# wadewilliamsw1234/Multi-level-Indoor-SLAM

Hardware: AMD Instinct MI355X
Metric: keyframes gated/sec (VPR+kNN+LightGlue verify) (higher is better)
Workload: dtype bf16

## Files before the change

include/mlgate.h:

```cpp
#ifndef MLGATE_H
#define MLGATE_H

#include <stddef.h>
#include <stdint.h>

#ifdef __cplusplus
extern "C" {
#endif

#define MLG_OK 0
#define MLG_EINVAL (-1)
#define MLG_EHIP (-2)
#define MLG_ENOMEM (-3)

#define MLG_VIT_DEPTH 12
#define MLG_VIT_EMBED 768
#define MLG_VIT_PATCH_K 768

#define MLG_ABI_VERSION 3
#define MLG_STRUCT_INIT(T) {(uint32_t)sizeof(T), (uint32_t)MLG_ABI_VERSION}
int mlg_abi_version(void);
const char* mlg_strerror(int status);

typedef struct mlg_vit_block {
// ... 274 lines not shown
                             void* stream);
int mlg_op_mixvpr_head(const mlg_mixvpr_weights* w, const float* features, int B, float* desc, void* stream);

typedef struct mlg_sp_weights {
    uint32_t struct_size, abi_version;
    const float* conv1a_w;
    const float* conv1a_b;
    const uint16_t* w[11];
    const float* b[11];
} mlg_sp_weights;
size_t mlg_superpoint_workspace_bytes(int B, int H, int W);
int mlg_superpoint(const mlg_sp_weights* w, const uint8_t* frames, int B, int H, int W, int C, long frame_stride,
                   float detection_threshold, int max_keypoints, int nms_radius, int remove_borders, void* workspace,
                   size_t workspace_bytes, float* keypoints, float* scores, float* descriptors,
                   uint16_t* descriptors_bf16, int32_t* counts, void* stream);

typedef struct mlg_lg_block {
    const uint16_t* Wqkv; const float* bqkv;
    const uint16_t* Wout; const float* bout;
    const uint16_t* Wf1;  const float* bf1;
    const float* ln_g;    const float* ln_b;
    const uint16_t* Wf2;  const float* bf2;
} mlg_lg_block;
typedef struct mlg_lg_weights {
    uint32_t struct_size, abi_version;
    const float* Wr;
    mlg_lg_block self[9], cross[9];
    const uint16_t* Wfinal[9]; const float* bfinal[9];
    const float* wmatch[9];    const float* bmatch[9];
    const float* wconf[8];     const float* bconf[8];
// ... 131 lines not shown
```

multi-level-indoor-slam_amd/csrc/abi.cpp:

```cpp
#include <hip/hip_runtime.h>

#include <math.h>

#include <mutex>
#include <vector>

#include "../../include/mlgate.h"
#include <cstddef>

#include "common.h"
#include "kernels.h"
#include "ws_carve.h"

namespace {

constexpr int PATCH = 14;

struct VitGeom {
    int B, S, grid, P, T, Tpad, E, heads;
    explicit VitGeom(int b, int s, int e = MLG_VIT_EMBED)
        : B(b), S(s), grid(s / PATCH), P(grid * grid), T(grid * grid + 1), E(e), heads(e / 64) {
        Tpad = (T + 63) / 64 * 64;
    }
};
// ... 585 lines not shown
                                s));
    return mlg_mixvpr_head(*w, feat, B, desc, s);
}

int mlg_op_mixvpr_preprocess(const uint8_t* frames, int B, int H, int W, int C, long frame_stride, float* out,
                             void* stream) {
    return mlg_mixvpr_preprocess(frames, B, H, W, C, frame_stride, out, (hipStream_t)stream);
}

int mlg_op_mixvpr_head(const mlg_mixvpr_weights* w, const float* features, int B, float* desc, void* stream) {
    if (!mlg_head_ok(w, MLG_ABI_VERSION) || !mixvpr_head_ok(w)) return MLG_EINVAL;
    return mlg_mixvpr_head(*w, features, B, desc, (hipStream_t)stream);
}

size_t mlg_superpoint_workspace_bytes(int B, int H, int W) { return mlg_superpoint_ws_bytes(B, H, W); }

int mlg_superpoint(const mlg_sp_weights* w, const uint8_t* frames, int B, int H, int W, int C, long frame_stride,
                   float detection_threshold, int max_keypoints, int nms_radius, int remove_borders, void* workspace,
                   size_t workspace_bytes, float* keypoints, float* scores, float* descriptors,
                   uint16_t* descriptors_bf16, int32_t* counts, void* stream) {
    if (!mlg_head_ok(w, MLG_ABI_VERSION) || !frames || !workspace || !keypoints || !scores || !descriptors || !counts)
        return MLG_EINVAL;
    if (!w->conv1a_w || !w->conv1a_b) return MLG_EINVAL;
    for (int i = 0; i < 11; ++i) {
        if (!w->w[i] || !w->b[i]) return MLG_EINVAL;
        if ((reinterpret_cast<uintptr_t>(w->w[i]) & 15) || (reinterpret_cast<uintptr_t>(w->b[i]) & 15))
            return MLG_EINVAL;
    }
    if (frame_stride < (long)H * W * C) return MLG_EINVAL;
    return mlg_superpoint_run(*w, frames, B, H, W, C, frame_stride, detection_threshold, max_keypoints, nms_radius,
// ... 264 lines not shown
```

multi-level-indoor-slam_amd/csrc/kernels.h:

```cpp
#pragma once
#include <hip/hip_runtime.h>
#include <stddef.h>
#include <stdint.h>

#include <algorithm>

#include "../../include/mlgate.h"

typedef uint16_t bf16_t;

template <class T>
inline bool mlg_head_ok(const T* p, uint32_t abi_version) {
    return p && p->struct_size == (uint32_t)sizeof(T) && p->abi_version == abi_version;
}

#define MLG_PROF_SLOTS 9
struct MlgProfScope {
    int slot;
    hipStream_t s;
    double work;
    hipEvent_t a = nullptr, b = nullptr;
    MlgProfScope(int slot, hipStream_t s, double work);
    ~MlgProfScope();
};
// ... 102 lines not shown
size_t mlg_proximity_ws_bytes(int N, int nrows);
int mlg_proximity_count_run(const double* pos, const int64_t* floor, int N, int row0, int nrows, double radius,
                            int min_gap, int strict, void* ws, size_t ws_bytes, long long* totals, hipStream_t s);
int mlg_proximity_emit_run(const double* pos, const int64_t* floor, int N, int row0, int nrows, double radius,
                           int min_gap, int strict, const void* ws, size_t ws_bytes, int32_t* pairs, double* dist,
                           uint8_t* valid, hipStream_t s);

size_t mlg_ransac_ws_bytes(int P, long S_total, int H);
int mlg_ransac_run(const float* kp1, const float* kp2, const int32_t* offs, int P, long S_total, const double* K,
                   int k_stride, double thr, int H, uint64_t seed, void* ws, size_t ws_bytes, double* model_out,
                   uint8_t* mask, int32_t* inliers, double* pose, int32_t* status, hipStream_t s);
int mlg_recover_pose_run(const float* kp1, const float* kp2, const int32_t* offs, int P, const double* K,
                         int k_stride, const double* E, const uint8_t* mask, double* pose, hipStream_t s);

size_t mlg_superpoint_ws_bytes(int B, int H, int W);
int mlg_superpoint_run(const mlg_sp_weights& w, const uint8_t* frames, int B, int H, int W, int C, long frame_stride,
                       float det_thr, int max_kp, int nms_radius, int border, void* ws, size_t ws_bytes, float* kpts,
                       float* kscores, float* desc, uint16_t* desc_bf16, int32_t* count, hipStream_t s);

struct mlg_lg_conf_i {
    const int* rowseg;
    const float* wc; const float* bc;
    const float* wm; const float* bm;
    float thr, width;
    float* lz; uint8_t* flags;
};
int mlg_lg_ffn(const bf16_t* ctx, float* X, bf16_t* xcopy, int ldc, int M, const mlg_lg_block& w, hipStream_t s,
               const mlg_lg_conf_i* conf = nullptr, int relu = 0);
int mlg_lg_proj(bool self_block, const bf16_t* xcopy, int ldx, const bf16_t* W, const float* bias, const float* efac,
                const uint8_t* live, bf16_t* Q, bf16_t* K, bf16_t* Vt, int Npad, hipStream_t s);
// ... 42 lines not shown
```

multi-level-indoor-slam_amd/csrc/superpoint.hip:

```cpp
#include "common.h"
#include "kernels.h"
#include "model_shapes.h"
#include "ws_carve.h"

namespace {

constexpr int TS = 16;
constexpr int HALO = TS + 2;
constexpr int KC = 64;

__global__ __launch_bounds__(256) void k_sp_conv1a(const uint8_t* __restrict__ frames, long frame_stride, int H, int W,
                                                   int C, const float* __restrict__ w, const float* __restrict__ b,
                                                   bf16_t* __restrict__ out) {
    __shared__ float g[HALO][HALO];
    __shared__ float sw[64 * 9 + 64];
    const int bz = blockIdx.z;
    const int y0 = blockIdx.y * TS, x0 = blockIdx.x * TS;
    const uint8_t* img = frames + (size_t)bz * frame_stride;
    for (int i = threadIdx.x; i < 64 * 9; i += 256) sw[i] = w[i];
    if (threadIdx.x < 64) sw[576 + threadIdx.x] = b[threadIdx.x];
    for (int i = threadIdx.x; i < HALO * HALO; i += 256) {
        const int yy = y0 - 1 + i / HALO, xx = x0 - 1 + i % HALO;
        float v = 0.f;
        if (yy >= 0 && yy < H && xx >= 0 && xx < W) {
// ... 243 lines not shown
    const long i = (long)blockIdx.x * blockDim.x + threadIdx.x;
    if (i < n) mask[i] = mask[i] | ((ss[i] == mp[i]) & !supp[i]);
}
__global__ void k_nms_final(float* __restrict__ s, const uint8_t* __restrict__ mask, int B, int H, int W,
                            int border) {
    const long i = (long)blockIdx.x * blockDim.x + threadIdx.x;
    if (i >= (long)B * H * W) return;
    const int x = (int)(i % W), y = (int)((i / W) % H);
    float v = mask[i] ? s[i] : 0.f;
    if (y < border || x < border || y >= H - border || x >= W - border) v = -1.f;
    s[i] = v;
}

constexpr int NMS_TH = 32, NMS_TW = 64, NMS_HALO = 20;
constexpr int NMS_LH = NMS_TH + 2 * NMS_HALO, NMS_LW = NMS_TW + 2 * NMS_HALO, NMS_N = NMS_LH * NMS_LW;

template <typename T> struct Vec4;
template <> struct Vec4<float> { typedef float4 type; };
template <> struct Vec4<uint8_t> { typedef uchar4 type; };

template <typename T>
__device__ __forceinline__ T vmax_(T a, T b) { return a > b ? a : b; }
template <>
__device__ __forceinline__ float vmax_(float a, float b) { return fmaxf(a, b); }

template <int M, typename T>
__device__ __forceinline__ void nms_pool4(const T* in, T* tmp, T* out, T lo) {
    typedef typename Vec4<T>::type V;
    constexpr int GX = NMS_LW / 4, GY = NMS_LH / 4;
    constexpr int XR0 = M > 4 ? M - 4 : 0, XR1 = M > 4 ? NMS_LH - M + 4 : NMS_LH;
    constexpr int XG0 = M / 4, XGN = GX - 2 * (M / 4);
    for (int i = threadIdx.x; i < (XR1 - XR0) * XGN; i += blockDim.x) {
        const int y = XR0 + i / XGN, g = XG0 + i % XGN;
        const V* row = reinterpret_cast<const V*>(in + y * NMS_LW);
        const V c = row[g];
        const V l = g > 0 ? row[g - 1] : V{lo, lo, lo, lo};
        const V r = g + 1 < GX ? row[g + 1] : V{lo, lo, lo, lo};
        const T v[12] = {l.x, l.y, l.z, l.w, c.x, c.y, c.z, c.w, r.x, r.y, r.z, r.w};
        T o[4];
#pragma unroll
        for (int k = 0; k < 4; ++k) {
            T m = v[k];
#pragma unroll
            for (int d = 1; d <= 8; ++d) m = vmax_(m, v[k + d]);
            o[k] = m;
        }
        reinterpret_cast<V*>(tmp + y * NMS_LW)[g] = V{o[0], o[1], o[2], o[3]};
    }
    __syncthreads();
    constexpr int YG0 = M / 4, YGN = GY - 2 * (M / 4), YC0 = M, YCN = NMS_LW - 2 * M;
    for (int i = threadIdx.x; i < YGN * YCN; i += blockDim.x) {
        const int g = YG0 + i / YCN, x = YC0 + i % YCN, y0 = 4 * g;
        T v[12];
#pragma unroll
        for (int k = 0; k < 12; ++k) {
            const int y = y0 - 4 + k;
            v[k] = (y >= 0 && y < NMS_LH) ? tmp[y * NMS_LW + x] : lo;
        }
#pragma unroll
        for (int k = 0; k < 4; ++k) {
            T m = v[k];
#pragma unroll
            for (int d = 1; d <= 8; ++d) m = vmax_(m, v[k + d]);
            out[(y0 + k) * NMS_LW + x] = m;
        }
    }
    __syncthreads();
}

__global__ __launch_bounds__(512) void k_sp_nms(const float* __restrict__ sc, float* __restrict__ out, int B, int H,
                                                int W, int border) {
    __shared__ __attribute__((aligned(16))) char nms_smem[(size_t)NMS_N * (4 * 4 + 3)];
    float* S = reinterpret_cast<float*>(nms_smem);
    float* A = S + NMS_N;
    float* Tm = A + NMS_N;
    float* P = Tm + NMS_N;
    uint8_t* MK = reinterpret_cast<uint8_t*>(P + NMS_N);
    uint8_t* SP = MK + NMS_N;
    uint8_t* TU = SP + NMS_N;
    const int tx = blockIdx.x, ty = blockIdx.y, b = blockIdx.z;
    const int ox = tx * NMS_TW - NMS_HALO, oy = ty * NMS_TH - NMS_HALO;
    const float* img = sc + (size_t)b * H * W;
    auto inside = [&](int i) {
        const int y = i / NMS_LW + oy, x = i % NMS_LW + ox;
        return y >= 0 && y < H && x >= 0 && x < W;
    };
    for (int i = threadIdx.x; i < NMS_N; i += blockDim.x) {
        const int y = i / NMS_LW + oy, x = i % NMS_LW + ox;
        S[i] = (y >= 0 && y < H && x >= 0 && x < W) ? img[(size_t)y * W + x] : -INFINITY;
    }
    __syncthreads();
    nms_pool4<4>(S, Tm, P, -INFINITY);
    for (int i = threadIdx.x; i < NMS_N; i += blockDim.x) MK[i] = inside(i) && S[i] == P[i];
    __syncthreads();
    auto iteration = [&](auto m) {
        constexpr int MS = decltype(m)::value;
        nms_pool4<MS + 4>(MK, TU, SP, (uint8_t)0);
        for (int i = threadIdx.x; i < NMS_N; i += blockDim.x) A[i] = inside(i) ? (SP[i] ? 0.f : S[i]) : -INFINITY;
        __syncthreads();
        nms_pool4<MS + 8>(A, Tm, P, -INFINITY);
        for (int i = threadIdx.x; i < NMS_N; i += blockDim.x)
            MK[i] = MK[i] | (inside(i) && A[i] == P[i] && !SP[i]);
        __syncthreads();
    };
    iteration(std::integral_constant<int, 4>{});
    iteration(std::integral_constant<int, 12>{});
    for (int i = threadIdx.x; i < NMS_TH * NMS_TW; i += blockDim.x) {
        const int ly = i / NMS_TW + NMS_HALO, lx = i % NMS_TW + NMS_HALO;
        const int y = ly + oy, x = lx + ox;
        if (y >= H || x >= W) continue;
        const int l = ly * NMS_LW + lx;
        float v = MK[l] ? S[l] : 0.f;
        if (y < border || x < border || y >= H - border || x >= W - border) v = -1.f;
        out[(size_t)b * H * W + (size_t)y * W + x] = v;
    }
}

constexpr int SEL_T = 1024;
constexpr int SEL_KMAX = 4096;

__global__ __launch_bounds__(SEL_T) void k_sp_select(const float* __restrict__ scores, int H, int W, float thr, int k,
                                                     uint32_t* __restrict__ cand_key, int32_t* __restrict__ cand_idx,
                                                     float* __restrict__ kpts, float* __restrict__ kscore,
                                                     int32_t* __restrict__ count) {
    const int b = blockIdx.x, tid = threadIdx.x;
    const long HW = (long)H * W;
    const float* s = scores + b * HW;
    uint32_t* ck = cand_key + b * HW;
    int32_t* ci = cand_idx + b * HW;
    __shared__ int scan[SEL_T];
    __shared__ uint32_t hist[256];
    __shared__ unsigned long long keys[SEL_KMAX];
    __shared__ int sh_n, sh_gt;
    __shared__ uint32_t sh_prefix;

    __shared__ int wsum[2][SEL_T / 64];
    const int lane = tid & 63, wave = tid >> 6;
    constexpr int PER = 16, CH = SEL_T * PER;
    const bool vec = (HW & 3) == 0;
    int base = 0;
    for (long c0 = 0, it = 0; c0 < HW; c0 += CH, ++it) {
        const long p0 = c0 + (long)tid * PER;
        float v[PER];
#pragma unroll
        for (int q = 0; q < PER / 4; ++q) {
            const long i = p0 + 4 * q;
            if (vec && i + 3 < HW) {
                const float4 f = *reinterpret_cast<const float4*>(s + i);
                v[4 * q] = f.x; v[4 * q + 1] = f.y; v[4 * q + 2] = f.z; v[4 * q + 3] = f.w;
            } else {
#pragma unroll
                for (int j = 0; j < 4; ++j) v[4 * q + j] = i + j < HW ? s[i + j] : -INFINITY;
            }
        }
        int cnt = 0;
#pragma unroll
        for (int j = 0; j < PER; ++j) cnt += v[j] > thr;
        int x = cnt;
#pragma unroll
        for (int o = 1; o < 64; o <<= 1) {
            const int y = __shfl_up(x, o, 64);
            if (lane >= o) x += y;
        }
        if (lane == 63) wsum[it & 1][wave] = x;
        __syncthreads();
        int wbase = 0, tot = 0;
#pragma unroll
        for (int w = 0; w < SEL_T / 64; ++w) {
            const int t = wsum[it & 1][w];
            wbase += w < wave ? t : 0;
            tot += t;
        }
        int off = base + wbase + x - cnt;
#pragma unroll
        for (int j = 0; j < PER; ++j)
            if (v[j] > thr) {
                ck[off] = __float_as_uint(v[j]);
                ci[off] = (int32_t)(p0 + j);
                ++off;
            }
        base += tot;
    }
    if (tid == 0) sh_n = base;
    __syncthreads();
    const int n = sh_n;
    float* kp = kpts + (size_t)b * k * 2;
    float* ks = kscore + (size_t)b * k;
    if (n <= k) {
        for (int i = tid; i < n; i += SEL_T) {
            const int idx = ci[i];
            kp[2 * i] = (float)(idx % W);
            kp[2 * i + 1] = (float)(idx / W);
            ks[i] = __uint_as_float(ck[i]);
        }
        if (tid == 0) count[b] = n;
        return;
    }
    uint32_t prefix = 0, pmask = 0;
    int want = k;
    for (int pass = 0; pass < 4; ++pass) {
        const int shift = 24 - 8 * pass;
        if (tid < 256) hist[tid] = 0;
        __syncthreads();
        for (int i = tid; i < n; i += SEL_T) {
            const uint32_t key = ck[i];
            if ((key & pmask) == prefix) atomicAdd(&hist[(key >> shift) & 255], 1u);
        }
        __syncthreads();
        if (tid == 0) {
            int acc = 0, d = 255;
            for (; d > 0; --d) {
                if (acc + (int)hist[d] >= want) break;
                acc += hist[d];
            }
            sh_prefix = prefix | ((uint32_t)d << shift);
            sh_gt = acc;
        }
        __syncthreads();
        want -= sh_gt;
        prefix = sh_prefix;
        pmask |= 255u << shift;
        __syncthreads();
    }
    const uint32_t T = prefix;
    if (tid == 0) sh_gt = 0;
    __syncthreads();
    int gt = 0;
    for (int i = tid; i < n; i += SEL_T) gt += ck[i] > T;
    atomicAdd(&sh_gt, gt);
    __syncthreads();
    const int need_eq = k - sh_gt;
    const int seg2 = (n + SEL_T - 1) / SEL_T;
    const int b0 = tid * seg2, b1 = min(n, b0 + seg2);
    int e = 0;
    for (int i = b0; i < b1; ++i) e += ck[i] == T;
    scan[tid] = e;
    __syncthreads();
    for (int o = 1; o < SEL_T; o <<= 1) {
        const int v = tid >= o ? scan[tid - o] : 0;
        __syncthreads();
        scan[tid] += v;
        __syncthreads();
    }
    if (tid == 0) sh_n = 0;
    __syncthreads();
    int erank = scan[tid] - e;
    for (int i = b0; i < b1; ++i) {
        const uint32_t key = ck[i];
        bool take = key > T;
        if (key == T) {
            take = erank < need_eq;
            ++erank;
        }
        if (take) {
            const int slot = atomicAdd(&sh_n, 1);
            keys[slot] = ((unsigned long long)key << 32) | (uint32_t)(~(uint32_t)ci[i]);
        }
    }
    __syncthreads();
    int np2 = 1;
    while (np2 < k) np2 <<= 1;
    for (int i = k + tid; i < np2; i += SEL_T) keys[i] = 0ull;
    __syncthreads();
    for (int size = 2; size <= np2; size <<= 1)
        for (int stride = size >> 1; stride > 0; stride >>= 1) {
            for (int i = tid; i < np2; i += SEL_T) {
                const int j = i ^ stride;
                if (j > i) {
                    const bool desc = (i & size) == 0;
                    const unsigned long long a = keys[i], bq = keys[j];
                    if ((a < bq) == desc) { keys[i] = bq; keys[j] = a; }
                }
            }
            __syncthreads();
        }
    for (int i = tid; i < k; i += SEL_T) {
        const unsigned long long v = keys[i];
        const int idx = (int)(~(uint32_t)(v & 0xffffffffu));
        kp[2 * i] = (float)(idx % W);
        kp[2 * i + 1] = (float)(idx / W);
        ks[i] = __uint_as_float((uint32_t)(v >> 32));
    }
    if (tid == 0) count[b] = k;
}

__device__ __forceinline__ float4 cell_normed(const float* __restrict__ d, const float* __restrict__ bias, int lane,
                                              bool valid) {
    if (!valid) return make_float4(0.f, 0.f, 0.f, 0.f);
    float4 v = *reinterpret_cast<const float4*>(d + lane * 4);
    const float4 bb = *reinterpret_cast<const float4*>(bias + lane * 4);
// ... 79 lines not shown
template <int L>
int gemm_layer(const mlg_sp_weights& w, const bf16_t* in, float* out, int M, hipStream_t s) {
    constexpr SpLayer l = SP_LAYERS[L];
    static_assert(l.k == 1, "gemm_layer is the 1 x 1 kernel");
    return mlg_gemm_f32out(in, w.w[L], out, M, l.cout, l.cin, s);
}

struct SpBufs {
    bf16_t *A, *Bf;
    float *logits, *dmap, *sc;
    float *t0, *t1;
    uint8_t* mask;
    uint8_t *u0, *u1;
    uint32_t* ckey;
    int32_t* cidx;
};

size_t sp_carve(int B, int H, int W, void* base, SpBufs* out) {
    WsCarver c(base);
    SpBufs b;
    const size_t n = (size_t)B * H * W, cells = (size_t)H * W / 64;
    b.A = c.take<bf16_t>(n * 64);
    b.Bf = c.take<bf16_t>(n * 64);
    b.logits = c.take<float>(B * cells * 128);
    b.dmap = c.take<float>(B * cells * 256);
    b.sc = c.take<float>(n);
    b.t0 = c.take<float>(2 * n);
    b.t1 = b.t0 ? b.t0 + n : nullptr;
    b.mask = c.take<uint8_t>(n);
    b.u0 = c.take<uint8_t>(2 * n);
    b.u1 = b.u0 ? b.u0 + n : nullptr;
    b.ckey = c.take<uint32_t>(n);
    b.cidx = c.take<int32_t>(n);
    if (out) *out = b;
    return c.total();
}

}

size_t mlg_superpoint_ws_bytes(int B, int H, int W) {
    if (B <= 0 || H < 16 || W < 16) return 0;
    return sp_carve(B, H, W, nullptr, nullptr);
}

int mlg_superpoint_run(const mlg_sp_weights& w, const uint8_t* frames, int B, int H, int W, int C, long frame_stride,
                       float det_thr, int max_kp, int nms_radius, int border, void* ws, size_t ws_bytes, float* kpts,
                       float* kscores, float* desc, uint16_t* desc_bf16, int32_t* count, hipStream_t s) {
    if (B <= 0 || H < 16 || W < 16 || (C != 1 && C != 3 && C != 4) || max_kp <= 0 ||
        max_kp > SEL_KMAX || nms_radius < 0 || border < 0)
        return MLG_EINVAL;
    SpBufs b;
    if (sp_carve(B, H, W, ws, &b) > ws_bytes) return MLG_EINVAL;
// ... 7 lines not shown
    MLG_TRY((conv_layer<1, false>(w, b.Bf, b.A, B, h, wd, s)));
    MLG_TRY((conv_layer<2, true>(w, b.A, b.Bf, B, h, wd, s)));
    h /= 2; wd /= 2;
    MLG_TRY((conv_layer<3, false>(w, b.Bf, b.A, B, h, wd, s)));
    MLG_TRY((conv_layer<4, true>(w, b.A, b.Bf, B, h, wd, s)));
    h /= 2; wd /= 2;
    MLG_TRY((conv_layer<5, false>(w, b.Bf, b.A, B, h, wd, s)));
    MLG_TRY((conv_layer<6, false>(w, b.A, b.Bf, B, h, wd, s)));
    const int M = B * h * wd;
    bf16_t* cPa = b.A;
    bf16_t* cDa = b.A + (size_t)M * SP_LAYERS[7].cout;
    MLG_TRY((conv_layer<7, false>(w, b.Bf, cPa, B, h, wd, s)));
    MLG_TRY((conv_layer<9, false>(w, b.Bf, cDa, B, h, wd, s)));
    MLG_TRY((gemm_layer<8>(w, cPa, b.logits, M, s)));
    MLG_TRY((gemm_layer<10>(w, cDa, b.dmap, M, s)));
    hipLaunchKernelGGL(k_sp_scores, dim3((M + 255) / 256), dim3(256), 0, s, b.logits, 128, w.b[8], B, h, wd, b.sc);
    MLG_LAUNCH_CHECK();
    H = 8 * h;
    W = 8 * wd;
    const float* nms_out = b.sc;
    if (nms_radius == 4) {
        hipLaunchKernelGGL(k_sp_nms, dim3((unsigned)((W + NMS_TW - 1) / NMS_TW), (unsigned)((H + NMS_TH - 1) / NMS_TH),
                                          (unsigned)B),
                           dim3(512), 0, s, b.sc, b.t0, B, H, W, border);
        MLG_LAUNCH_CHECK();
        nms_out = b.t0;
    } else {
        const long n = (long)B * H * W;
        const dim3 g((unsigned)((n + 255) / 256)), t(256);
        auto maxpool_f = [&](const float* in, float* out) {
            hipLaunchKernelGGL(k_maxfilt<float>, g, t, 0, s, in, b.t1, B, H, W, nms_radius, 0);
            hipLaunchKernelGGL(k_maxfilt<float>, g, t, 0, s, (const float*)b.t1, out, B, H, W, nms_radius, 1);
        };
        maxpool_f(b.sc, b.t0);
        hipLaunchKernelGGL(k_nms_init, g, t, 0, s, b.sc, b.t0, b.mask, n);
        for (int it = 0; it < 2; ++it) {
            hipLaunchKernelGGL(k_maxfilt<uint8_t>, g, t, 0, s, b.mask, b.u1, B, H, W, nms_radius, 0);
            hipLaunchKernelGGL(k_maxfilt<uint8_t>, g, t, 0, s, (const uint8_t*)b.u1, b.u0, B, H, W, nms_radius, 1);
            hipLaunchKernelGGL(k_nms_supp, g, t, 0, s, b.sc, b.u0, b.t0, n);
            hipLaunchKernelGGL(k_maxfilt<float>, g, t, 0, s, (const float*)b.t0, b.t1, B, H, W, nms_radius, 0);
            float* mp = (float*)b.ckey;
            hipLaunchKernelGGL(k_maxfilt<float>, g, t, 0, s, (const float*)b.t1, mp, B, H, W, nms_radius, 1);
            hipLaunchKernelGGL(k_nms_update, g, t, 0, s, b.t0, mp, b.u0, b.mask, n);
        }
        hipLaunchKernelGGL(k_nms_final, g, t, 0, s, b.sc, b.mask, B, H, W, border);
        MLG_LAUNCH_CHECK();
    }
    hipLaunchKernelGGL(k_sp_select, dim3(B), dim3(SEL_T), 0, s, nms_out, H, W, det_thr, max_kp, b.ckey, b.cidx, kpts,
                       kscores, count);
    MLG_LAUNCH_CHECK();
    hipLaunchKernelGGL(k_sp_desc, dim3((unsigned)(((long)B * max_kp + 3) / 4)), dim3(256), 0, s, b.dmap, w.b[10], B, h,
                       wd, kpts, count, max_kp, desc, desc_bf16);
    MLG_LAUNCH_CHECK();
    return MLG_OK;
}
```

multi-level-indoor-slam_amd/mlgate/_native.py:

```python
import ctypes
import os

_HERE = os.path.dirname(os.path.abspath(__file__))
LIB_PATH = os.path.join(_HERE, "libmlgate.so")
TORCH_LIB_PATH = os.path.join(_HERE, "libmlgate_torch.so")
OPS = ("vit_forward_into", "dino_forward_into", "dino_weights_check", "salad_forward", "knn_gate", "knn_query", "row_normalize", "similarity", "xcorr_score", "xcorr_batch", "rerank_gate", "seq_gate",
       "knn_append", "superpoint",
       "lightglue", "ransac_epipolar", "recover_pose", "resnet50", "loftr_features", "loftr_pack_tails", "loftr_coarse_layer", "loftr_match", "superglue", "pillow_resize_224", "plane_ransac", "proximity",
       "jpeg_pixels", "mixvpr_forward", "mixvpr_head", "mixvpr_preprocess", "vlad", "anyloc_forward", "kmeans_step",
       "crica_forward", "vit_trunk", "crica_pool", "crica_encoder",
       "weights_check", "prof_enable", "prof_reset", "prof_read")


c_int, c_long, c_size_t, c_float, c_double, c_void_p = (
    ctypes.c_int, ctypes.c_long, ctypes.c_size_t, ctypes.c_float, ctypes.c_double, ctypes.c_void_p)

EXPORTS = {
    "mlg_abi_version": (c_int, []),
    "mlg_strerror": (ctypes.c_char_p, [c_int]),
    "mlg_vit_workspace_bytes": (c_size_t, [c_int, c_int]),
    "mlg_vit_forward": (c_int, [c_void_p, c_void_p, c_int, c_int, c_int, c_int, c_long, c_int, c_int, c_void_p,
                                c_size_t, c_void_p, c_void_p, c_void_p]),
    "mlg_dino_workspace_bytes": (c_size_t, [c_int, c_int, c_int]),
    "mlg_dino_forward": (c_int, [c_void_p, c_void_p, c_int, c_int, c_int, c_int, c_long, c_int, c_int, c_void_p,
# ... 42 lines not shown
    "mlg_anyloc_workspace_bytes": (c_size_t, [c_int, c_int, c_int]),
    "mlg_anyloc_forward": (c_int, [c_void_p, c_void_p, c_void_p, c_int, c_int, c_int, c_int, c_long, c_int, c_int,
                                   c_void_p, c_size_t, c_void_p, c_void_p]),
    "mlg_kmeans_workspace_bytes": (c_size_t, [c_long, c_int]),
    "mlg_kmeans_step": (c_int, [c_void_p, c_long, c_void_p, c_int, c_void_p, c_void_p, c_void_p, c_void_p, c_size_t,
                                c_void_p]),
    "mlg_crica_forward": (c_int, [c_void_p, c_void_p, c_void_p, c_int, c_int, c_int, c_int, c_long, c_int, c_int,
                                  c_int, c_void_p, c_size_t, c_void_p, c_void_p, c_void_p]),
    "mlg_op_vit_trunk": (c_int, [c_void_p, c_void_p, c_int, c_int, c_int, c_int, c_long, c_int, c_int, c_void_p,
                                 c_size_t, c_void_p, c_void_p]),
    "mlg_op_crica_pool": (c_int, [c_void_p, c_void_p, c_void_p, c_int, c_int, c_float, c_void_p, c_void_p]),
    "mlg_op_crica_encoder": (c_int, [c_void_p, c_void_p, c_int, c_int, c_void_p, c_size_t, c_void_p, c_void_p]),
    "mlg_superpoint_workspace_bytes": (c_size_t, [c_int, c_int, c_int]),
    "mlg_superpoint": (c_int, [c_void_p, c_void_p, c_int, c_int, c_int, c_int, c_long, c_float, c_int, c_int, c_int,
                               c_void_p, c_size_t, c_void_p, c_void_p, c_void_p, c_void_p, c_void_p, c_void_p]),
    "mlg_lightglue_workspace_bytes": (c_size_t, [c_int, c_int]),
    "mlg_lightglue": (c_int, [c_void_p, c_void_p, c_void_p, c_void_p, c_int, c_int, c_void_p, c_void_p, c_int,
                              c_float, c_float, c_float, c_int, c_void_p, c_size_t, c_void_p, c_void_p, c_void_p,
                              c_void_p, c_void_p]),
    "mlg_op_gemm_f32out": (c_int, [c_void_p, c_void_p, c_void_p, c_int, c_int, c_int, c_void_p]),
    "mlg_op_gemm_f32out_variant": (c_int, [c_int, c_void_p, c_void_p, c_void_p, c_int, c_int, c_int, c_void_p]),
    "mlg_set_gemm_variant": (c_int, [c_int]),
    "mlg_set_loftr_similarity": (c_int, [c_int]),
    "mlg_op_gemm_bias_gelu": (c_int, [c_void_p, c_void_p, c_void_p, c_void_p, c_int, c_int, c_int, c_void_p]),
    "mlg_op_gemm_residual": (c_int, [c_void_p, c_void_p, c_void_p, c_void_p, c_void_p, c_int, c_int, c_int,
                                     c_void_p]),
    "mlg_op_gemm_residual_split": (c_int, [c_void_p, c_void_p, c_void_p, c_void_p, c_void_p, c_int, c_int, c_int,
                                           c_void_p]),
    "mlg_op_gemm_bias_gelu_split": (c_int, [c_void_p, c_void_p, c_void_p, c_void_p, c_int, c_int, c_int, c_void_p]),
    "mlg_op_layernorm_bf16": (c_int, [c_void_p, c_void_p, c_void_p, c_void_p, c_int, c_void_p]),
# ... 144 lines not shown
```

Measured before the change: 551.7.

## Fuse SuperPoint softmax, NMS and candidate emission into one tiled kernel

```diff
diff --git a/include/mlgate.h b/include/mlgate.h
--- a/include/mlgate.h
+++ b/include/mlgate.h
@@ -312,6 +312,7 @@
                    float detection_threshold, int max_keypoints, int nms_radius, int remove_borders, void* workspace,
                    size_t workspace_bytes, float* keypoints, float* scores, float* descriptors,
                    uint16_t* descriptors_bf16, int32_t* counts, void* stream);
+int mlg_set_superpoint_tail(int tail);
 
 typedef struct mlg_lg_block {
     const uint16_t* Wqkv; const float* bqkv;
diff --git a/multi-level-indoor-slam_amd/csrc/abi.cpp b/multi-level-indoor-slam_amd/csrc/abi.cpp
--- a/multi-level-indoor-slam_amd/csrc/abi.cpp
+++ b/multi-level-indoor-slam_amd/csrc/abi.cpp
@@ -623,6 +623,7 @@
 }
 
 size_t mlg_superpoint_workspace_bytes(int B, int H, int W) { return mlg_superpoint_ws_bytes(B, H, W); }
+int mlg_set_superpoint_tail(int tail) { return mlg_superpoint_set_tail(tail); }
 
 int mlg_superpoint(const mlg_sp_weights* w, const uint8_t* frames, int B, int H, int W, int C, long frame_stride,
                    float detection_threshold, int max_keypoints, int nms_radius, int remove_borders, void* workspace,
diff --git a/multi-level-indoor-slam_amd/csrc/kernels.h b/multi-level-indoor-slam_amd/csrc/kernels.h
--- a/multi-level-indoor-slam_amd/csrc/kernels.h
+++ b/multi-level-indoor-slam_amd/csrc/kernels.h
@@ -140,6 +140,7 @@
                          int k_stride, const double* E, const uint8_t* mask, double* pose, hipStream_t s);
 
 size_t mlg_superpoint_ws_bytes(int B, int H, int W);
+int mlg_superpoint_set_tail(int tail);
 int mlg_superpoint_run(const mlg_sp_weights& w, const uint8_t* frames, int B, int H, int W, int C, long frame_stride,
                        float det_thr, int max_kp, int nms_radius, int border, void* ws, size_t ws_bytes, float* kpts,
                        float* kscores, float* desc, uint16_t* desc_bf16, int32_t* count, hipStream_t s);
diff --git a/multi-level-indoor-slam_amd/csrc/superpoint.hip b/multi-level-indoor-slam_amd/csrc/superpoint.hip
--- a/multi-level-indoor-slam_amd/csrc/superpoint.hip
+++ b/multi-level-indoor-slam_amd/csrc/superpoint.hip
@@ -281,6 +281,11 @@
 
 constexpr int NMS_TH = 32, NMS_TW = 64, NMS_HALO = 20;
 constexpr int NMS_LH = NMS_TH + 2 * NMS_HALO, NMS_LW = NMS_TW + 2 * NMS_HALO, NMS_N = NMS_LH * NMS_LW;
+static_assert(NMS_HALO % 8 == 4 && NMS_TH % 8 == 0 && NMS_TW % 8 == 0, "cells of a tile");
+constexpr int NMS_CH = NMS_LH / 8 + 1, NMS_CW = NMS_LW / 8 + 1, NMS_CELLS = NMS_CH * NMS_CW;
+constexpr size_t NMS_LDS_BYTES = (size_t)NMS_N * (4 + 4 + 1 + 1);
+static_assert(NMS_LDS_BYTES + 2 * NMS_CELLS * 4 + 64 <= 80 * 1024, "two workgroups per CU");
+static_assert((size_t)NMS_TH * NMS_TW * 8 <= (size_t)NMS_N * 4, "candidate staging fits the scratch plane");
 
 template <typename T> struct Vec4;
 template <> struct Vec4<float> { typedef float4 type; };
@@ -291,18 +296,17 @@
 template <>
 __device__ __forceinline__ float vmax_(float a, float b) { return fmaxf(a, b); }
 
-template <int M, typename T>
-__device__ __forceinline__ void nms_pool4(const T* in, T* tmp, T* out, T lo) {
+template <int M, typename T, typename Load, typename Emit>
+__device__ __forceinline__ void nms_pool4(Load load, T* tmp, T lo, Emit emit) {
     typedef typename Vec4<T>::type V;
     constexpr int GX = NMS_LW / 4, GY = NMS_LH / 4;
     constexpr int XR0 = M > 4 ? M - 4 : 0, XR1 = M > 4 ? NMS_LH - M + 4 : NMS_LH;
     constexpr int XG0 = M / 4, XGN = GX - 2 * (M / 4);
     for (int i = threadIdx.x; i < (XR1 - XR0) * XGN; i += blockDim.x) {
         const int y = XR0 + i / XGN, g = XG0 + i % XGN;
-        const V* row = reinterpret_cast<const V*>(in + y * NMS_LW);
-        const V c = row[g];
-        const V l = g > 0 ? row[g - 1] : V{lo, lo, lo, lo};
-        const V r = g + 1 < GX ? row[g + 1] : V{lo, lo, lo, lo};
+        const V c = load(y, g);
+        const V l = g > 0 ? load(y, g - 1) : V{lo, lo, lo, lo};
+        const V r = g + 1 < GX ? load(y, g + 1) : V{lo, lo, lo, lo};
         const T v[12] = {l.x, l.y, l.z, l.w, c.x, c.y, c.z, c.w, r.x, r.y, r.z, r.w};
         T o[4];
 #pragma unroll
@@ -329,49 +333,106 @@
             T m = v[k];
 #pragma unroll
             for (int d = 1; d <= 8; ++d) m = vmax_(m, v[k + d]);
-            out[(y0 + k) * NMS_LW + x] = m;
+            emit(y0 + k, x, m);
         }
     }
     __syncthreads();
 }
 
-__global__ __launch_bounds__(512) void k_sp_nms(const float* __restrict__ sc, float* __restrict__ out, int B, int H,
-                                                int W, int border) {
-    __shared__ __attribute__((aligned(16))) char nms_smem[(size_t)NMS_N * (4 * 4 + 3)];
+template <bool LOGITS, bool EMIT>
+__global__ __launch_bounds__(512, 2) void k_sp_nms(const float* __restrict__ src, int ld,
+                                                   const float* __restrict__ bias, float* __restrict__ out, int B,
+                                                   int H, int W, int border, float thr,
+                                                   uint32_t* __restrict__ cand_key, int32_t* __restrict__ cand_idx,
+                                                   int32_t* __restrict__ cand_n) {
+    __shared__ __attribute__((aligned(16))) char nms_smem[NMS_LDS_BYTES];
+    __shared__ float cmx[NMS_CELLS], csum[NMS_CELLS];
+    __shared__ int sh_cand, sh_base;
     float* S = reinterpret_cast<float*>(nms_smem);
-    float* A = S + NMS_N;
-    float* Tm = A + NMS_N;
-    float* P = Tm + NMS_N;
-    uint8_t* MK = reinterpret_cast<uint8_t*>(P + NMS_N);
+    float* T = S + NMS_N;
+    uint8_t* TU = reinterpret_cast<uint8_t*>(T);
+    uint8_t* MK = reinterpret_cast<uint8_t*>(T + NMS_N);
     uint8_t* SP = MK + NMS_N;
-    uint8_t* TU = SP + NMS_N;
     const int tx = blockIdx.x, ty = blockIdx.y, b = blockIdx.z;
     const int ox = tx * NMS_TW - NMS_HALO, oy = ty * NMS_TH - NMS_HALO;
-    const float* img = sc + (size_t)b * H * W;
-    auto inside = [&](int i) {
-        const int y = i / NMS_LW + oy, x = i % NMS_LW + ox;
+    if (threadIdx.x == 0) sh_cand = 0;
+    if (LOGITS) {
+        const int Hc = H / 8, Wc = W / 8, cy0 = oy >> 3, cx0 = ox >> 3;
+        const float* lg = src + (size_t)b * Hc * Wc * ld;
+        if (threadIdx.x < NMS_CELLS) {
+            const int cy = cy0 + threadIdx.x / NMS_CW, cx = cx0 + threadIdx.x % NMS_CW;
+            if (cy >= 0 && cy < Hc && cx >= 0 && cx < Wc) {
+                const float* l = lg + ((size_t)cy * Wc + cx) * ld;
+                float v[65];
+                float mx = -INFINITY;
+#pragma unroll
+                for (int c = 0; c < 65; ++c) {
+                    v[c] = l[c] + bias[c];
+                    mx = fmaxf(mx, v[c]);
+                }
+                float s = 0.f;
+#pragma unroll
+                for (int c = 0; c < 65; ++c) {
+                    v[c] = expf(v[c] - mx);
+                    s += v[c];
+                }
+                cmx[threadIdx.x] = mx;
+                csum[threadIdx.x] = s;
+            }
+        }
+        __syncthreads();
+        for (int i = threadIdx.x; i < NMS_CELLS * 64; i += blockDim.x) {
+            const int cell = i >> 6, c = i & 63;
+            const int cy = cy0 + cell / NMS_CW, cx = cx0 + cell % NMS_CW;
+            const int ly = cy * 8 + (c >> 3) - oy, lx = cx * 8 + (c & 7) - ox;
+            if (ly < 0 || ly >= NMS_LH || lx < 0 || lx >= NMS_LW) continue;
+            float sc = -INFINITY;
+            if (cy >= 0 && cy < Hc && cx >= 0 && cx < Wc) {
+                const float v = lg[((size_t)cy * Wc + cx) * ld + c] + bias[c];
+                sc = expf(v - cmx[cell]) / csum[cell];
+            }
+            S[ly * NMS_LW + lx] = sc;
+        }
+    } else {
+        const float* img = src + (size_t)b * H * W;
+        for (int i = threadIdx.x; i < NMS_N; i += blockDim.x) {
+            const int y = i / NMS_LW + oy, x = i % NMS_LW + ox;
+            S[i] = (y >= 0 && y < H && x >= 0 && x < W) ? img[(size_t)y * W + x] : -INFINITY;
+        }
+    }
+    __syncthreads();
+    auto inside = [&](int ly, int lx) {
+        const int y = ly + oy, x = lx + ox;
         return y >= 0 && y < H && x >= 0 && x < W;
     };
-    for (int i = threadIdx.x; i < NMS_N; i += blockDim.x) {
-        const int y = i / NMS_LW + oy, x = i % NMS_LW + ox;
-        S[i] = (y >= 0 && y < H && x >= 0 && x < W) ? img[(size_t)y * W + x] : -INFINITY;
-    }
-    __syncthreads();
-    nms_pool4<4>(S, Tm, P, -INFINITY);
-    for (int i = threadIdx.x; i < NMS_N; i += blockDim.x) MK[i] = inside(i) && S[i] == P[i];
-    __syncthreads();
+    auto load_s = [&](int y, int g) { return reinterpret_cast<const float4*>(S + y * NMS_LW)[g]; };
+    auto load_mk = [&](int y, int g) { return reinterpret_cast<const uchar4*>(MK + y * NMS_LW)[g]; };
+    auto load_a = [&](int y, int g) {
+        float4 s = load_s(y, g);
+        const uchar4 p = reinterpret_cast<const uchar4*>(SP + y * NMS_LW)[g];
+        const int lx = 4 * g;
+        if (p.x && inside(y, lx)) s.x = 0.f;
+        if (p.y && inside(y, lx + 1)) s.y = 0.f;
+        if (p.z && inside(y, lx + 2)) s.z = 0.f;
+        if (p.w && inside(y, lx + 3)) s.w = 0.f;
+        return s;
+    };
+    nms_pool4<4, float>(load_s, T, -INFINITY, [&](int y, int x, float m) {
+        const int l = y * NMS_LW + x;
+        MK[l] = inside(y, x) && S[l] == m;
+    });
     auto iteration = [&](auto m) {
         constexpr int MS = decltype(m)::value;
-        nms_pool4<MS + 4>(MK, TU, SP, (uint8_t)0);
-        for (int i = threadIdx.x; i < NMS_N; i += blockDim.x) A[i] = inside(i) ? (SP[i] ? 0.f : S[i]) : -INFINITY;
-        __syncthreads();
-        nms_pool4<MS + 8>(A, Tm, P, -INFINITY);
-        for (int i = threadIdx.x; i < NMS_N; i += blockDim.x)
-            MK[i] = MK[i] | (inside(i) && A[i] == P[i] && !SP[i]);
-        __syncthreads();
+        nms_pool4<MS + 4, uint8_t>(load_mk, TU, (uint8_t)0,
+                                   [&](int y, int x, uint8_t mm) { SP[y * NMS_LW + x] = mm; });
+        nms_pool4<MS + 8, float>(load_a, T, -INFINITY, [&](int y, int x, float mm) {
+            const int l = y * NMS_LW + x;
+            MK[l] = MK[l] | (inside(y, x) && !SP[l] && S[l] == mm);
+        });
     };
     iteration(std::integral_constant<int, 4>{});
     iteration(std::integral_constant<int, 12>{});
+    uint2* stage = reinterpret_cast<uint2*>(T);
     for (int i = threadIdx.x; i < NMS_TH * NMS_TW; i += blockDim.x) {
         const int ly = i / NMS_TW + NMS_HALO, lx = i % NMS_TW + NMS_HALO;
         const int y = ly + oy, x = lx + ox;
@@ -379,155 +440,35 @@
         const int l = ly * NMS_LW + lx;
         float v = MK[l] ? S[l] : 0.f;
         if (y < border || x < border || y >= H - border || x >= W - border) v = -1.f;
-        out[(size_t)b * H * W + (size_t)y * W + x] = v;
+        if (EMIT) {
+            if (v > thr) stage[atomicAdd(&sh_cand, 1)] = make_uint2(__float_as_uint(v), (uint32_t)(y * W + x));
+        } else {
+            out[(size_t)b * H * W + (size_t)y * W + x] = v;
+        }
+    }
+    if (EMIT) {
+        __syncthreads();
+        const int n = sh_cand;
+        if (threadIdx.x == 0 && n > 0) sh_base = atomicAdd(&cand_n[b], n);
+        __syncthreads();
+        if (n > 0) {
+            const size_t base = (size_t)b * H * W + sh_base;
+            for (int i = threadIdx.x; i < n; i += blockDim.x) {
+                cand_key[base + i] = stage[i].x;
+                cand_idx[base + i] = (int32_t)stage[i].y;
+            }
+        }
     }
 }
 
 constexpr int SEL_T = 1024;
 constexpr int SEL_KMAX = 4096;
 
-__global__ __launch_bounds__(SEL_T) void k_sp_select(const float* __restrict__ scores, int H, int W, float thr, int k,
-                                                     uint32_t* __restrict__ cand_key, int32_t* __restrict__ cand_idx,
-                                                     float* __restrict__ kpts, float* __restrict__ kscore,
-                                                     int32_t* __restrict__ count) {
-    const int b = blockIdx.x, tid = threadIdx.x;
-    const long HW = (long)H * W;
-    const float* s = scores + b * HW;
-    uint32_t* ck = cand_key + b * HW;
-    int32_t* ci = cand_idx + b * HW;
-    __shared__ int scan[SEL_T];
-    __shared__ uint32_t hist[256];
-    __shared__ unsigned long long keys[SEL_KMAX];
-    __shared__ int sh_n, sh_gt;
-    __shared__ uint32_t sh_prefix;
-
-    __shared__ int wsum[2][SEL_T / 64];
-    const int lane = tid & 63, wave = tid >> 6;
-    constexpr int PER = 16, CH = SEL_T * PER;
-    const bool vec = (HW & 3) == 0;
-    int base = 0;
-    for (long c0 = 0, it = 0; c0 < HW; c0 += CH, ++it) {
-        const long p0 = c0 + (long)tid * PER;
-        float v[PER];
-#pragma unroll
-        for (int q = 0; q < PER / 4; ++q) {
-            const long i = p0 + 4 * q;
-            if (vec && i + 3 < HW) {
-                const float4 f = *reinterpret_cast<const float4*>(s + i);
-                v[4 * q] = f.x; v[4 * q + 1] = f.y; v[4 * q + 2] = f.z; v[4 * q + 3] = f.w;
-            } else {
-#pragma unroll
-                for (int j = 0; j < 4; ++j) v[4 * q + j] = i + j < HW ? s[i + j] : -INFINITY;
-            }
-        }
-        int cnt = 0;
-#pragma unroll
-        for (int j = 0; j < PER; ++j) cnt += v[j] > thr;
-        int x = cnt;
-#pragma unroll
-        for (int o = 1; o < 64; o <<= 1) {
-            const int y = __shfl_up(x, o, 64);
-            if (lane >= o) x += y;
-        }
-        if (lane == 63) wsum[it & 1][wave] = x;
-        __syncthreads();
-        int wbase = 0, tot = 0;
-#pragma unroll
-        for (int w = 0; w < SEL_T / 64; ++w) {
-            const int t = wsum[it & 1][w];
-            wbase += w < wave ? t : 0;
-            tot += t;
-        }
-        int off = base + wbase + x - cnt;
-#pragma unroll
-        for (int j = 0; j < PER; ++j)
-            if (v[j] > thr) {
-                ck[off] = __float_as_uint(v[j]);
-                ci[off] = (int32_t)(p0 + j);
-                ++off;
-            }
-        base += tot;
-    }
-    if (tid == 0) sh_n = base;
-    __syncthreads();
-    const int n = sh_n;
-    float* kp = kpts + (size_t)b * k * 2;
-    float* ks = kscore + (size_t)b * k;
-    if (n <= k) {
-        for (int i = tid; i < n; i += SEL_T) {
-            const int idx = ci[i];
-            kp[2 * i] = (float)(idx % W);
-            kp[2 * i + 1] = (float)(idx / W);
-            ks[i] = __uint_as_float(ck[i]);
-        }
-        if (tid == 0) count[b] = n;
-        return;
-    }
-    uint32_t prefix = 0, pmask = 0;
-    int want = k;
-    for (int pass = 0; pass < 4; ++pass) {
-        const int shift = 24 - 8 * pass;
-        if (tid < 256) hist[tid] = 0;
-        __syncthreads();
-        for (int i = tid; i < n; i += SEL_T) {
-            const uint32_t key = ck[i];
-            if ((key & pmask) == prefix) atomicAdd(&hist[(key >> shift) & 255], 1u);
-        }
-        __syncthreads();
-        if (tid == 0) {
-            int acc = 0, d = 255;
-            for (; d > 0; --d) {
-                if (acc + (int)hist[d] >= want) break;
-                acc += hist[d];
-            }
-            sh_prefix = prefix | ((uint32_t)d << shift);
-            sh_gt = acc;
-        }
-        __syncthreads();
-        want -= sh_gt;
-        prefix = sh_prefix;
-        pmask |= 255u << shift;
-        __syncthreads();
-    }
-    const uint32_t T = prefix;
-    if (tid == 0) sh_gt = 0;
-    __syncthreads();
-    int gt = 0;
-    for (int i = tid; i < n; i += SEL_T) gt += ck[i] > T;
-    atomicAdd(&sh_gt, gt);
-    __syncthreads();
-    const int need_eq = k - sh_gt;
-    const int seg2 = (n + SEL_T - 1) / SEL_T;
-    const int b0 = tid * seg2, b1 = min(n, b0 + seg2);
-    int e = 0;
-    for (int i = b0; i < b1; ++i) e += ck[i] == T;
-    scan[tid] = e;
-    __syncthreads();
-    for (int o = 1; o < SEL_T; o <<= 1) {
-        const int v = tid >= o ? scan[tid - o] : 0;
-        __syncthreads();
-        scan[tid] += v;
-        __syncthreads();
-    }
-    if (tid == 0) sh_n = 0;
-    __syncthreads();
-    int erank = scan[tid] - e;
-    for (int i = b0; i < b1; ++i) {
-        const uint32_t key = ck[i];
-        bool take = key > T;
-        if (key == T) {
-            take = erank < need_eq;
-            ++erank;
-        }
-        if (take) {
-            const int slot = atomicAdd(&sh_n, 1);
-            keys[slot] = ((unsigned long long)key << 32) | (uint32_t)(~(uint32_t)ci[i]);
-        }
-    }
-    __syncthreads();
+__device__ __forceinline__ void sel_sort_desc(unsigned long long* keys, int n) {
+    const int tid = threadIdx.x;
     int np2 = 1;
-    while (np2 < k) np2 <<= 1;
-    for (int i = k + tid; i < np2; i += SEL_T) keys[i] = 0ull;
+    while (np2 < n) np2 <<= 1;
+    for (int i = n + tid; i < np2; i += SEL_T) keys[i] = 0ull;
     __syncthreads();
     for (int size = 2; size <= np2; size <<= 1)
         for (int stride = size >> 1; stride > 0; stride >>= 1) {
@@ -541,6 +482,140 @@
             }
             __syncthreads();
         }
+}
+
+template <bool LIST>
+__global__ __launch_bounds__(SEL_T) void k_sp_select(const float* __restrict__ scores,
+                                                     const int32_t* __restrict__ cand_n, int H, int W, float thr,
+                                                     int k, uint32_t* __restrict__ cand_key,
+                                                     int32_t* __restrict__ cand_idx, float* __restrict__ kpts,
+                                                     float* __restrict__ kscore, int32_t* __restrict__ count) {
+    const int b = blockIdx.x, tid = threadIdx.x;
+    const long HW = (long)H * W;
+    uint32_t* ck = cand_key + b * HW;
+    int32_t* ci = cand_idx + b * HW;
+    __shared__ uint32_t hist[256];
+    __shared__ unsigned long long keys[SEL_KMAX];
+    __shared__ int sh_n, sh_gt;
+    __shared__ unsigned long long sh_prefix;
+    int n;
+    if (LIST) {
+        n = cand_n[b];
+    } else {
+        const float* s = scores + b * HW;
+        __shared__ int wsum[2][SEL_T / 64];
+        const int lane = tid & 63, wave = tid >> 6;
+        constexpr int PER = 16, CH = SEL_T * PER;
+        const bool vec = (HW & 3) == 0;
+        int base = 0;
+        for (long c0 = 0, it = 0; c0 < HW; c0 += CH, ++it) {
+            const long p0 = c0 + (long)tid * PER;
+            float v[PER];
+#pragma unroll
+            for (int q = 0; q < PER / 4; ++q) {
+                const long i = p0 + 4 * q;
+                if (vec && i + 3 < HW) {
+                    const float4 f = *reinterpret_cast<const float4*>(s + i);
+                    v[4 * q] = f.x; v[4 * q + 1] = f.y; v[4 * q + 2] = f.z; v[4 * q + 3] = f.w;
+                } else {
+#pragma unroll
+                    for (int j = 0; j < 4; ++j) v[4 * q + j] = i + j < HW ? s[i + j] : -INFINITY;
+                }
+            }
+            int cnt = 0;
+#pragma unroll
+            for (int j = 0; j < PER; ++j) cnt += v[j] > thr;
+            int x = cnt;
+#pragma unroll
+            for (int o = 1; o < 64; o <<= 1) {
+                const int y = __shfl_up(x, o, 64);
+                if (lane >= o) x += y;
+            }
+            if (lane == 63) wsum[it & 1][wave] = x;
+            __syncthreads();
+            int wbase = 0, tot = 0;
+#pragma unroll
+            for (int w = 0; w < SEL_T / 64; ++w) {
+                const int t = wsum[it & 1][w];
+                wbase += w < wave ? t : 0;
+                tot += t;
+            }
+            int off = base + wbase + x - cnt;
+#pragma unroll
+            for (int j = 0; j < PER; ++j)
+                if (v[j] > thr) {
+                    ck[off] = __float_as_uint(v[j]);
+                    ci[off] = (int32_t)(p0 + j);
+                    ++off;
+                }
+            base += tot;
+        }
+        if (tid == 0) sh_n = base;
+        __syncthreads();
+        n = sh_n;
+    }
+    float* kp = kpts + (size_t)b * k * 2;
+    float* ks = kscore + (size_t)b * k;
+    auto sort_key = [&](int i) { return ((unsigned long long)ck[i] << 32) | (uint32_t)(~(uint32_t)ci[i]); };
+    if (n <= k) {
+        if (LIST) {
+            for (int i = tid; i < n; i += SEL_T)
+                keys[i] = ((unsigned long long)(~(uint32_t)ci[i]) << 32) | ck[i];
+            __syncthreads();
+            sel_sort_desc(keys, n);
+            for (int i = tid; i < n; i += SEL_T) {
+                const unsigned long long v = keys[i];
+                const int idx = (int)(~(uint32_t)(v >> 32));
+                kp[2 * i] = (float)(idx % W);
+                kp[2 * i + 1] = (float)(idx / W);
+                ks[i] = __uint_as_float((uint32_t)(v & 0xffffffffu));
+            }
+        } else {
+            for (int i = tid; i < n; i += SEL_T) {
+                const int idx = ci[i];
+                kp[2 * i] = (float)(idx % W);
+                kp[2 * i + 1] = (float)(idx / W);
+                ks[i] = __uint_as_float(ck[i]);
+            }
+        }
+        if (tid == 0) count[b] = n;
+        return;
+    }
+    unsigned long long prefix = 0, pmask = 0;
+    int want = k;
+    for (int pass = 0; pass < 8; ++pass) {
+        const int shift = 56 - 8 * pass;
+        if (tid < 256) hist[tid] = 0;
+        __syncthreads();
+        for (int i = tid; i < n; i += SEL_T) {
+            const unsigned long long key = sort_key(i);
+            if ((key & pmask) == prefix) atomicAdd(&hist[(uint32_t)(key >> shift) & 255], 1u);
+        }
+        __syncthreads();
+        if (tid == 0) {
+            int acc = 0, d = 255;
+            for (; d > 0; --d) {
+                if (acc + (int)hist[d] >= want) break;
+                acc += hist[d];
+            }
+            sh_prefix = prefix | ((unsigned long long)d << shift);
+            sh_gt = acc;
+        }
+        __syncthreads();
+        want -= sh_gt;
+        prefix = sh_prefix;
+        pmask |= 255ull << shift;
+        __syncthreads();
+    }
+    const unsigned long long T = prefix;
+    if (tid == 0) sh_n = 0;
+    __syncthreads();
+    for (int i = tid; i < n; i += SEL_T) {
+        const unsigned long long key = sort_key(i);
+        if (key >= T) keys[atomicAdd(&sh_n, 1)] = key;
+    }
+    __syncthreads();
+    sel_sort_desc(keys, k);
     for (int i = tid; i < k; i += SEL_T) {
         const unsigned long long v = keys[i];
         const int idx = (int)(~(uint32_t)(v & 0xffffffffu));
@@ -650,6 +725,7 @@
     uint8_t *u0, *u1;
     uint32_t* ckey;
     int32_t* cidx;
+    int32_t* ccnt;
 };
 
 size_t sp_carve(int B, int H, int W, void* base, SpBufs* out) {
@@ -668,10 +744,19 @@
     b.u1 = b.u0 ? b.u0 + n : nullptr;
     b.ckey = c.take<uint32_t>(n);
     b.cidx = c.take<int32_t>(n);
+    b.ccnt = reinterpret_cast<int32_t*>(b.sc);
     if (out) *out = b;
     return c.total();
 }
 
+int g_tail = 0;
+
+}
+
+int mlg_superpoint_set_tail(int tail) {
+    if (tail != 0 && tail != 1) return MLG_EINVAL;
+    g_tail = tail;
+    return MLG_OK;
 }
 
 size_t mlg_superpoint_ws_bytes(int B, int H, int W) {
@@ -709,41 +794,51 @@
     MLG_TRY((conv_layer<9, false>(w, b.Bf, cDa, B, h, wd, s)));
     MLG_TRY((gemm_layer<8>(w, cPa, b.logits, M, s)));
     MLG_TRY((gemm_layer<10>(w, cDa, b.dmap, M, s)));
-    hipLaunchKernelGGL(k_sp_scores, dim3((M + 255) / 256), dim3(256), 0, s, b.logits, 128, w.b[8], B, h, wd, b.sc);
-    MLG_LAUNCH_CHECK();
     H = 8 * h;
     W = 8 * wd;
-    const float* nms_out = b.sc;
-    if (nms_radius == 4) {
-        hipLaunchKernelGGL(k_sp_nms, dim3((unsigned)((W + NMS_TW - 1) / NMS_TW), (unsigned)((H + NMS_TH - 1) / NMS_TH),
-                                          (unsigned)B),
-                           dim3(512), 0, s, b.sc, b.t0, B, H, W, border);
+    const dim3 nms_grid((unsigned)((W + NMS_TW - 1) / NMS_TW), (unsigned)((H + NMS_TH - 1) / NMS_TH), (unsigned)B);
+    if (nms_radius == 4 && g_tail == 0) {
+        if (hipMemsetAsync(b.ccnt, 0, sizeof(int32_t) * B, s) != hipSuccess) return MLG_EHIP;
+        hipLaunchKernelGGL((k_sp_nms<true, true>), nms_grid, dim3(512), 0, s, b.logits, 128, w.b[8], nullptr, B, H, W,
+                           border, det_thr, b.ckey, b.cidx, b.ccnt);
         MLG_LAUNCH_CHECK();
-        nms_out = b.t0;
+        hipLaunchKernelGGL(k_sp_select<true>, dim3(B), dim3(SEL_T), 0, s, nullptr, b.ccnt, H, W, det_thr, max_kp,
+                           b.ckey, b.cidx, kpts, kscores, count);
+        MLG_LAUNCH_CHECK();
     } else {
-        const long n = (long)B * H * W;
-        const dim3 g((unsigned)((n + 255) / 256)), t(256);
-        auto maxpool_f = [&](const float* in, float* out) {
-            hipLaunchKernelGGL(k_maxfilt<float>, g, t, 0, s, in, b.t1, B, H, W, nms_radius, 0);
-            hipLaunchKernelGGL(k_maxfilt<float>, g, t, 0, s, (const float*)b.t1, out, B, H, W, nms_radius, 1);
-        };
-        maxpool_f(b.sc, b.t0);
-        hipLaunchKernelGGL(k_nms_init, g, t, 0, s, b.sc, b.t0, b.mask, n);
-        for (int it = 0; it < 2; ++it) {
-            hipLaunchKernelGGL(k_maxfilt<uint8_t>, g, t, 0, s, b.mask, b.u1, B, H, W, nms_radius, 0);
-            hipLaunchKernelGGL(k_maxfilt<uint8_t>, g, t, 0, s, (const uint8_t*)b.u1, b.u0, B, H, W, nms_radius, 1);
-            hipLaunchKernelGGL(k_nms_supp, g, t, 0, s, b.sc, b.u0, b.t0, n);
-            hipLaunchKernelGGL(k_maxfilt<float>, g, t, 0, s, (const float*)b.t0, b.t1, B, H, W, nms_radius, 0);
-            float* mp = (float*)b.ckey;
-            hipLaunchKernelGGL(k_maxfilt<float>, g, t, 0, s, (const float*)b.t1, mp, B, H, W, nms_radius, 1);
-            hipLaunchKernelGGL(k_nms_update, g, t, 0, s, b.t0, mp, b.u0, b.mask, n);
-        }
-        hipLaunchKernelGGL(k_nms_final, g, t, 0, s, b.sc, b.mask, B, H, W, border);
+        hipLaunchKernelGGL(k_sp_scores, dim3((M + 255) / 256), dim3(256), 0, s, b.logits, 128, w.b[8], B, h, wd, b.sc);
         MLG_LAUNCH_CHECK();
-    }
-    hipLaunchKernelGGL(k_sp_select, dim3(B), dim3(SEL_T), 0, s, nms_out, H, W, det_thr, max_kp, b.ckey, b.cidx, kpts,
-                       kscores, count);
-    MLG_LAUNCH_CHECK();
+        const float* nms_out = b.sc;
+        if (nms_radius == 4) {
+            hipLaunchKernelGGL((k_sp_nms<false, false>), nms_grid, dim3(512), 0, s, b.sc, 0, nullptr, b.t0, B, H, W,
+                               border, det_thr, nullptr, nullptr, nullptr);
+            MLG_LAUNCH_CHECK();
+            nms_out = b.t0;
+        } else {
+            const long n = (long)B * H * W;
+            const dim3 g((unsigned)((n + 255) / 256)), t(256);
+            auto maxpool_f = [&](const float* in, float* out) {
+                hipLaunchKernelGGL(k_maxfilt<float>, g, t, 0, s, in, b.t1, B, H, W, nms_radius, 0);
+                hipLaunchKernelGGL(k_maxfilt<float>, g, t, 0, s, (const float*)b.t1, out, B, H, W, nms_radius, 1);
+            };
+            maxpool_f(b.sc, b.t0);
+            hipLaunchKernelGGL(k_nms_init, g, t, 0, s, b.sc, b.t0, b.mask, n);
+            for (int it = 0; it < 2; ++it) {
+                hipLaunchKernelGGL(k_maxfilt<uint8_t>, g, t, 0, s, b.mask, b.u1, B, H, W, nms_radius, 0);
+                hipLaunchKernelGGL(k_maxfilt<uint8_t>, g, t, 0, s, (const uint8_t*)b.u1, b.u0, B, H, W, nms_radius, 1);
+                hipLaunchKernelGGL(k_nms_supp, g, t, 0, s, b.sc, b.u0, b.t0, n);
+                hipLaunchKernelGGL(k_maxfilt<float>, g, t, 0, s, (const float*)b.t0, b.t1, B, H, W, nms_radius, 0);
+                float* mp = (float*)b.ckey;
+                hipLaunchKernelGGL(k_maxfilt<float>, g, t, 0, s, (const float*)b.t1, mp, B, H, W, nms_radius, 1);
+                hipLaunchKernelGGL(k_nms_update, g, t, 0, s, b.t0, mp, b.u0, b.mask, n);
+            }
+            hipLaunchKernelGGL(k_nms_final, g, t, 0, s, b.sc, b.mask, B, H, W, border);
+            MLG_LAUNCH_CHECK();
+        }
+        hipLaunchKernelGGL(k_sp_select<false>, dim3(B), dim3(SEL_T), 0, s, nms_out, nullptr, H, W, det_thr, max_kp,
+                           b.ckey, b.cidx, kpts, kscores, count);
+        MLG_LAUNCH_CHECK();
+    }
     hipLaunchKernelGGL(k_sp_desc, dim3((unsigned)(((long)B * max_kp + 3) / 4)), dim3(256), 0, s, b.dmap, w.b[10], B, h,
                        wd, kpts, count, max_kp, desc, desc_bf16);
     MLG_LAUNCH_CHECK();
diff --git a/multi-level-indoor-slam_amd/mlgate/_native.py b/multi-level-indoor-slam_amd/mlgate/_native.py
--- a/multi-level-indoor-slam_amd/mlgate/_native.py
+++ b/multi-level-indoor-slam_amd/mlgate/_native.py
@@ -80,6 +80,7 @@
     "mlg_superpoint_workspace_bytes": (c_size_t, [c_int, c_int, c_int]),
     "mlg_superpoint": (c_int, [c_void_p, c_void_p, c_int, c_int, c_int, c_int, c_long, c_float, c_int, c_int, c_int,
                                c_void_p, c_size_t, c_void_p, c_void_p, c_void_p, c_void_p, c_void_p, c_void_p]),
+    "mlg_set_superpoint_tail": (c_int, [c_int]),
     "mlg_lightglue_workspace_bytes": (c_size_t, [c_int, c_int]),
     "mlg_lightglue": (c_int, [c_void_p, c_void_p, c_void_p, c_void_p, c_int, c_int, c_void_p, c_void_p, c_int,
                               c_float, c_float, c_float, c_int, c_void_p, c_size_t, c_void_p, c_void_p, c_void_p,
```

Result: no change. 553.8 (median of 6 runs) (+0.4%).
